# facebookresearch/moolib

Measured on AMD Instinct MI355X. Metric: env frames/sec (whole node) IMPALA Atari-ResNet, higher is better.
Workload: dtype bf16; 1 GPU; model=IMPALA Atari deep ResNet (16/32/32ch, FC3872-256), global_batch=32, seq_len=20, parallelism=dp1, actor_batch_size=128, num_actor_batches=2, num_actor_cpus=10, virtual_batch_size=32, num_actions=18, frame=84x84x4 uint8

## Files before the change

### csrc/accumulator.cc

```cpp
#include "accumulator.h"

#include <ATen/Functions.h>
#include <c10/core/GradMode.h>

#include <cstdlib>
#include <sstream>

namespace mrl {

namespace {
struct NoGrad {
  c10::AutoGradMode g{false};
};
}

Accumulator::Ptr Accumulator::create(std::string name, std::vector<at::Tensor> params,
                                     std::vector<at::Tensor> buffers,
                                     std::shared_ptr<Group> group) {
  Ptr p(new Accumulator(std::move(name), std::move(params), std::move(buffers), std::move(group)));
  p->setup();
  return p;
}

Accumulator::Accumulator(std::string name, std::vector<at::Tensor> params,
                         std::vector<at::Tensor> buffers, std::shared_ptr<Group> group)
    : name_(std::move(name)),
      allParams_(std::move(params)),
      buffers_(std::move(buffers)),
      group_(std::move(group)) {
  rpc_ = group_->rpc();
  for (auto& p : allParams_) {
    if (p.requires_grad()) params_.push_back(p);
  }
  int64_t total = 0;
  for (auto& p : params_) {
    offsets_.push_back(total);
    numels_.push_back(p.numel());
    total += p.numel();
  }
  slots_.resize(1);
  slots_[0].flat = makeFlatLocked();
  if (const char* e = getenv("MOOLIB_AMD_MODEL_BCAST_S")) {
    modelBcastInterval_ = atof(e);
  }
}

at::Tensor Accumulator::makeFlatLocked() {
  NoGrad ng;
  int64_t total = offsets_.empty() ? 1 : offsets_.back() + numels_.back();
  auto opts = params_.empty()
                  ? at::TensorOptions().dtype(at::kFloat)
                  : at::TensorOptions().dtype(params_[0].scalar_type()).device(params_[0].device());
  return at::zeros({std::max<int64_t>(total, 1)}, opts);
}

Accumulator::~Accumulator() {
  if (rpc_ && !rpc_->isShutdown()) {
    rpc_->undefine(fn("reqmodel"));
    rpc_->undefine(fn("modelupd"));
    rpc_->undefine(fn("buffers"));
  }
}

void Accumulator::setup() {
  std::weak_ptr<Accumulator> weak = weak_from_this();

  rpc_->define(fn("reqmodel"), [weak](Frame f, const std::string& from, RespondFn respond) {
    if (auto self = weak.lock()) {
      std::lock_guard<std::mutex> lk(self->mu_);
      if (std::find(self->stateRequesters_.begin(), self->stateRequesters_.end(), from) ==
          self->stateRequesters_.end()) {
        self->stateRequesters_.push_back(from);
      }
    }
    respond("", {}, false);
  });

  rpc_->define(fn("modelupd"), [weak](Frame f, const std::string& from, RespondFn respond) {
    auto self = weak.lock();
    if (!self) {
      respond("accumulator gone", {}, true);
      return;
    }
    try {
      WireReader r(f.payload);
      int64_t version = r.i64();
      uint32_t nParams = r.u32();
      uint32_t nBuffers = r.u32();
      std::string statePayload(r.str());
      if (uint64_t(nParams) > f.tensors.size() || uint64_t(nBuffers) > f.tensors.size() ||
          uint64_t(nParams) + uint64_t(nBuffers) > f.tensors.size())
        throw RpcError("model update tensor shortfall");
      std::lock_guard<std::mutex> lk(self->mu_);
      self->pendingParams_.assign(f.tensors.begin(), f.tensors.begin() + nParams);
      self->pendingBuffers_.assign(f.tensors.begin() + nParams,
                                   f.tensors.begin() + nParams + nBuffers);
      self->pendingStateTensors_.assign(f.tensors.begin() + nParams + nBuffers, f.tensors.end());
      self->pendingStatePayload_ = std::move(statePayload);
      self->pendingVersion_ = version;
      self->havePendingModel_ = true;
      respond("", {}, false);
    } catch (const std::exception& e) {
      respond(e.what(), {}, true);
    }
  });

  rpc_->define(fn("buffers"), [weak](Frame f, const std::string& from, RespondFn respond) {
    if (auto self = weak.lock()) {
      std::lock_guard<std::mutex> lk(self->mu_);
      if (f.tensors.size() == self->buffers_.size()) {
        NoGrad ng;
        for (size_t i = 0; i < self->buffers_.size(); ++i) {
          if (self->buffers_[i].sizes() == f.tensors[i].sizes()) {
            self->buffers_[i].copy_(f.tensors[i]);
          }
        }
      }
    }
    respond("", {}, false);
  });
}

void Accumulator::connect(const std::string& addr) { rpc_->connect(addr); }

void Accumulator::resetLocked(const char* why) {
  MRL_LOG_INFO("accumulator '%s': reset (%s)", name_.c_str(), why);
  epoch_++;
  decided_ = false;
  hasGradients_ = false;
  results_.clear();
  slotCursor_ = 0;
  hookLaunchCounter_ = 0;
  hookLaunchedUpTo_ = 0;
  for (auto& s : slots_) {
    s.newBatch = s.newGrads = s.newSkipped = 0;
    s.totBatch = s.totGrads = s.totSkipped = 0;
    s.phase = GradPhase::wantDecision;
    s.hookPending = false;
    if (s.hookPoll) {
      drains_.push_back(std::move(s.hookPoll));
      s.hookPoll = nullptr;
      s.flat = makeFlatLocked();
    } else {
      NoGrad ng;
      s.flat.zero_();
    }
  }
  havePendingModel_ = false;
  hasNewState_ = false;
  stateRequesters_.clear();
  modelRequestSent_ = false;
  leader_.clear();
  isLeader_ = false;
}

void Accumulator::failAndResyncLocked(const char* why) {
  MRL_LOG_INFO("accumulator '%s': %s; resync", name_.c_str(), why);
  phase_ = Phase::inactive;
  syncSeen_ = 0;
  group_->requestResync();
}

void Accumulator::startElectionLocked() {
  phase_ = Phase::electing;
  ReduceValue v;
  v.kind = ReduceValue::leaderTuple;
  v.version = modelVersion_;
  v.leaderName = group_->myName();
  uint64_t epoch = epoch_;
  std::weak_ptr<Accumulator> weak = weak_from_this();
  group_->allReduce(fn("elect"), std::move(v), nullptr,
                    [weak, epoch](ReduceValue* rv, const std::string* err) {
                      auto self = weak.lock();
                      if (!self) return;
                      std::lock_guard<std::mutex> lk(self->mu_);
                      if (epoch != self->epoch_ || self->phase_ != Phase::electing) return;
                      if (err) {
                        self->failAndResyncLocked(("election failed: " + *err).c_str());
                        return;
                      }
                      self->leader_ = rv->leaderName;
                      self->isLeader_ = (rv->leaderName == self->group_->myName());
                      MRL_LOG_INFO("accumulator '%s': leader is '%s' (version %lld)%s",
                                   self->name_.c_str(), self->leader_.c_str(),
                                   (long long)rv->version, self->isLeader_ ? " - that's me" : "");
                      if (self->isLeader_) {
                        self->phase_ = Phase::running;
                      } else {
                        self->phase_ = Phase::fetching;
                        self->modelRequestSent_ = false;
                      }
                    });
}

void Accumulator::update() {
  group_->update();
  bool active = group_->active();
  uint64_t sid = group_->syncId();

  std::vector<std::function<bool()>> pollTombs;
  std::unique_lock<std::mutex> lk(mu_);
  for (auto it = drains_.begin(); it != drains_.end();) {
    bool done = true;
    try {
      done = (*it)();
    } catch (const std::exception& e) {
      MRL_LOG_ERROR("abandoned hook drain failed: %s", e.what());
    }
    if (done) {
      pollTombs.push_back(std::move(*it));
      it = drains_.erase(it);
    } else {
      ++it;
    }
  }

  if (!active) {
    if (phase_ != Phase::inactive) resetLocked("group inactive");
    phase_ = Phase::inactive;
    syncSeen_ = 0;
    return;
  }
  if (sid != syncSeen_) {
    syncSeen_ = sid;
    resetLocked("membership changed");
    startElectionLocked();
    return;
  }

  if (phase_ == Phase::fetching) {
    if (!modelRequestSent_ || secondsSince(fetchStarted_) > 5.0) {
      modelRequestSent_ = true;
      fetchStarted_ = now();
      std::string leader = leader_;
      rpc_->sendRequest(leader, fn("reqmodel"), "", {},
                        [](Frame* resp, const std::string* err) {
                          if (err) MRL_LOG_VERBOSE("requestModel failed: %s", err->c_str());
                        },
                        10.0);
    }
  }

  if (havePendingModel_ && (phase_ == Phase::fetching || phase_ == Phase::running)) {
    NoGrad ng;
    bool shapesOk = pendingParams_.size() == allParams_.size() &&
                    pendingBuffers_.size() == buffers_.size();
    if (shapesOk) {
      for (size_t i = 0; i < allParams_.size(); ++i) {
        allParams_[i].copy_(pendingParams_[i], true);
      }
      for (size_t i = 0; i < buffers_.size(); ++i) {
        buffers_[i].copy_(pendingBuffers_[i], true);
      }
      modelVersion_ = pendingVersion_;
      hasNewState_ = !pendingStatePayload_.empty() || !pendingStateTensors_.empty();
      phase_ = Phase::running;
      MRL_LOG_INFO("accumulator '%s': model adopted at version %lld", name_.c_str(),
                   (long long)modelVersion_);
    } else {
      MRL_LOG_ERROR("accumulator '%s': model update shape mismatch — ignored", name_.c_str());
    }
    havePendingModel_ = false;
    pendingParams_.clear();
    pendingBuffers_.clear();
  }

  if (phase_ == Phase::running) {
    for (auto& s : slots_) {
      if (s.phase == GradPhase::reducing && secondsSince(s.started) > 120.0) {
        MRL_LOG_ERROR("accumulator '%s': gradient reduce wedged >120s", name_.c_str());
        failAndResyncLocked("reduce wedged");
        return;
      }
    }
    GradSlot& cur = slots_[slotCursor_];
    if (cur.phase == GradPhase::wantDecision && decided_) {
      startCountRoundLocked();
    }
    tryLaunchHooksLocked();
    for (size_t si = 0; si < slots_.size(); ++si) {
      GradSlot& s = slots_[si];
      if (s.phase == GradPhase::reducing && s.hookPoll && !s.hookPending) {
        bool done = false;
        try {
          done = s.hookPoll();
        } catch (const std::exception& e) {
          pollTombs.push_back(std::move(s.hookPoll));
          s.hookPoll = nullptr;
          MRL_LOG_ERROR("local reduce hook poll failed: %s", e.what());
          failAndResyncLocked("hook poll failed");
          return;
        }
        if (done) {
          pollTombs.push_back(std::move(s.hookPoll));
          s.hookPoll = nullptr;
          NoGrad ng;
          at::Tensor result = s.flat.clone();
          completeSlotLocked(si, std::move(result));
        }
      }
    }
    applyPendingLocked();
    maybeSendModelUpdatesLocked();
  }
}

void Accumulator::startCountRoundLocked() {
  size_t si = slotCursor_;
  GradSlot& s = slots_[si];
  s.phase = GradPhase::counting;
  s.started = now();
  ReduceValue v;
  v.kind = ReduceValue::counts;
  v.batchSize = s.newBatch;
  v.numGradients = s.newGrads;
  v.numSkipped = s.newSkipped;
  s.newBatch = s.newGrads = s.newSkipped = 0;
  uint64_t epoch = epoch_;
  std::weak_ptr<Accumulator> weak = weak_from_this();
  group_->allReduce(
      fn("count") + "/" + std::to_string(si), std::move(v), nullptr,
      [weak, epoch, si](ReduceValue* rv, const std::string* err) {
        auto self = weak.lock();
        if (!self) return;
        std::lock_guard<std::mutex> lk(self->mu_);
        if (epoch != self->epoch_) return;
        GradSlot& s = self->slots_[si];
        if (s.phase != GradPhase::counting) return;
        if (err) {
          self->failAndResyncLocked(("count round failed: " + *err).c_str());
          return;
        }
        s.totBatch += rv->batchSize;
        s.totGrads += rv->numGradients;
        s.totSkipped += rv->numSkipped;
        self->decided_ = false;
        if (s.totBatch >= self->virtualBatchSize_ && s.totGrads > 0) {
          self->enterReducingLocked(si);
        } else {
          s.phase = GradPhase::wantDecision;
        }
      });
}

void Accumulator::enterReducingLocked(size_t si) {
  GradSlot& s = slots_[si];
  s.phase = GradPhase::reducing;
  s.started = now();
  slotCursor_ = (si + 1) % slots_.size();
  if (hook_) {
    s.launchSeq = hookLaunchCounter_++;
    s.hookPending = true;
    tryLaunchHooksLocked();
    return;
  }
  ReduceValue v;
  v.kind = ReduceValue::gradBundle;
  {
    NoGrad ng;
    v.tensors.push_back(s.flat.device().is_cpu() ? s.flat.clone() : s.flat.to(at::kCPU));
  }
  uint64_t epoch = epoch_;
  std::weak_ptr<Accumulator> weak = weak_from_this();
  group_->allReduce(
      fn("grads") + "/" + std::to_string(si), std::move(v), nullptr,
      [weak, epoch, si](ReduceValue* rv, const std::string* err) {
        auto self = weak.lock();
        if (!self) return;
        std::lock_guard<std::mutex> lk(self->mu_);
        if (epoch != self->epoch_) return;
        GradSlot& s = self->slots_[si];
        if (s.phase != GradPhase::reducing) return;
        if (err) {
          self->failAndResyncLocked(("gradient reduce failed: " + *err).c_str());
          return;
        }
        NoGrad ng;
        at::Tensor result = rv->tensors.at(0);
        if (!s.flat.device().is_cpu()) result = result.to(s.flat.device(), true);
        self->completeSlotLocked(si, std::move(result));
      });
}

void Accumulator::tryLaunchHooksLocked() {
  if (!hook_ || !drains_.empty()) return;
  for (size_t si = 0; si < slots_.size(); ++si) {
    GradSlot& s = slots_[si];
    if (s.phase == GradPhase::reducing && s.hookPending && s.launchSeq == hookLaunchedUpTo_) {
      s.hookPending = false;
      ++hookLaunchedUpTo_;
      try {
        s.hookPoll = hook_(s.flat);
      } catch (const std::exception& e) {
        MRL_LOG_ERROR("local reduce hook failed: %s", e.what());
        failAndResyncLocked("hook launch failed");
        return;
      }
    }
  }
}

void Accumulator::completeSlotLocked(size_t si, at::Tensor result) {
  GradSlot& s = slots_[si];
  results_.push_back(PendingResult{std::move(result), s.totBatch, s.totGrads, s.totSkipped});
  s.totBatch = s.totGrads = s.totSkipped = 0;
  s.phase = GradPhase::wantDecision;
  {
    NoGrad ng;
    s.flat.zero_();
  }
}

void Accumulator::applyPendingLocked() {
  if (hasGradients_ || results_.empty()) return;
  PendingResult r = std::move(results_.front());
  results_.pop_front();
  NoGrad ng;
  int64_t n = std::max<int64_t>(r.grads, 1);
  r.flat.div_(static_cast<double>(n));
  for (size_t i = 0; i < params_.size(); ++i) {
    auto& p = params_[i];
    at::Tensor slice = r.flat.narrow(0, offsets_[i], numels_[i]).view(p.sizes());
    if (!p.grad().defined()) {
      p.mutable_grad() = slice.clone();
    } else {
      p.grad().copy_(slice, true);
    }
  }
  statBatch_ = r.batch;
  statGrads_ = r.grads;
  statSkipped_ = r.skipped;
  modelVersion_ += 1;
  hasGradients_ = true;
}

void Accumulator::maybeSendModelUpdatesLocked() {
  if (!isLeader_) return;
  if (!buffers_.empty() && secondsSince(lastBuffersBroadcast_) >= 10.0) {
    lastBuffersBroadcast_ = now();
    std::vector<at::Tensor> cpuBuffers;
    {
      NoGrad ng;
      for (auto& b : buffers_) cpuBuffers.push_back(b.detach().to(at::kCPU));
    }
    for (auto& m : group_->members()) {
      if (m == group_->myName()) continue;
      rpc_->sendRequest(m, fn("buffers"), "", cpuBuffers,
                        [](Frame*, const std::string*) {}, 10.0);
    }
  }
  if (lastModelBroadcast_.time_since_epoch().count() == 0) lastModelBroadcast_ = now();
  if (secondsSince(lastModelBroadcast_) >= modelBcastInterval_) {
    lastModelBroadcast_ = now();
    std::vector<at::Tensor> frameTensors;
    {
      NoGrad ng;
      for (auto& p : allParams_) frameTensors.push_back(p.detach().to(at::kCPU));
      for (auto& b : buffers_) frameTensors.push_back(b.detach().to(at::kCPU));
    }
    WireWriter w;
    w.i64(modelVersion_);
    w.u32(static_cast<uint32_t>(allParams_.size()));
    w.u32(static_cast<uint32_t>(buffers_.size()));
    w.str("");
    for (auto& m : group_->members()) {
      if (m == group_->myName()) continue;
      rpc_->sendRequest(m, fn("modelupd"), w.out, frameTensors,
                        [](Frame*, const std::string*) {}, 30.0);
    }
  }
}

bool Accumulator::connected() {
  std::lock_guard<std::mutex> lk(mu_);
  return phase_ == Phase::running;
}

bool Accumulator::wantsState() {
  std::lock_guard<std::mutex> lk(mu_);
  return phase_ == Phase::running && isLeader_ && !stateRequesters_.empty();
}

bool Accumulator::hasNewState() {
  std::lock_guard<std::mutex> lk(mu_);
  return hasNewState_;
}

void Accumulator::setState(std::string payload, std::vector<at::Tensor> tensors) {
  std::vector<std::string> requesters;
  int64_t version;
  std::vector<at::Tensor> frameTensors;
  uint32_t nParams, nBuffers;
  {
    std::lock_guard<std::mutex> lk(mu_);
    requesters.swap(stateRequesters_);
    version = modelVersion_;
    NoGrad ng;
    for (auto& p : allParams_) frameTensors.push_back(p.detach().to(at::kCPU));
    for (auto& b : buffers_) frameTensors.push_back(b.detach().to(at::kCPU));
    nParams = static_cast<uint32_t>(allParams_.size());
    nBuffers = static_cast<uint32_t>(buffers_.size());
  }
  for (auto& t : tensors) frameTensors.push_back(t.device().is_cpu() ? t : t.to(at::kCPU));
  WireWriter w;
  w.i64(version);
  w.u32(nParams);
  w.u32(nBuffers);
  w.str(payload);
  for (auto& r : requesters) {
    rpc_->sendRequest(r, fn("modelupd"), w.out, frameTensors,
                      [r](Frame*, const std::string* err) {
                        if (err) {
                          MRL_LOG_INFO("model update to '%s' failed: %s", r.c_str(), err->c_str());
                        }
                      },
                      30.0);
  }
}

std::pair<std::string, std::vector<at::Tensor>> Accumulator::state() {
  std::lock_guard<std::mutex> lk(mu_);
  hasNewState_ = false;
  return {pendingStatePayload_, pendingStateTensors_};
}

bool Accumulator::wantsGradients() {
  std::lock_guard<std::mutex> lk(mu_);
  if (phase_ != Phase::running || decided_) return false;
  if (slots_[slotCursor_].phase != GradPhase::wantDecision) return false;
  size_t pending = results_.size() + (hasGradients_ ? 1 : 0);
  return pending < slots_.size();
}

bool Accumulator::hasGradients() {
  std::lock_guard<std::mutex> lk(mu_);
  return hasGradients_;
}

void Accumulator::skipGradients() {
  std::lock_guard<std::mutex> lk(mu_);
  if (phase_ != Phase::running || decided_) return;
  GradSlot& s = slots_[slotCursor_];
  if (s.phase != GradPhase::wantDecision) return;
  decided_ = true;
  s.newSkipped += 1;
}

void Accumulator::reduceGradients(int64_t batchSize) {
  std::lock_guard<std::mutex> lk(mu_);
  GradSlot& s = slots_[slotCursor_];
  if (phase_ != Phase::running || s.phase != GradPhase::wantDecision || decided_) {
    throw RpcError("reduce_gradients called when wants_gradients() is false");
  }
  NoGrad ng;
  std::vector<at::Tensor> slices, flatGrads, grads;
  slices.reserve(params_.size());
  flatGrads.reserve(params_.size());
  grads.reserve(params_.size());
  for (size_t i = 0; i < params_.size(); ++i) {
    auto& p = params_[i];
    if (p.grad().defined()) {
      slices.push_back(s.flat.narrow(0, offsets_[i], numels_[i]));
      flatGrads.push_back(p.grad().flatten());
      grads.push_back(p.grad());
    }
  }
  if (!grads.empty()) {
    at::_foreach_add_(slices, flatGrads);
    at::_foreach_zero_(grads);
  }
  decided_ = true;
  s.newBatch += batchSize;
  s.newGrads += 1;
}

void Accumulator::zeroGradients() {
  std::lock_guard<std::mutex> lk(mu_);
  NoGrad ng;
  std::vector<at::Tensor> grads;
  for (auto& p : params_) {
    if (p.grad().defined()) grads.push_back(p.grad());
  }
  if (!grads.empty()) at::_foreach_zero_(grads);
  hasGradients_ = false;
  applyPendingLocked();
}

int64_t Accumulator::modelVersion() {
  std::lock_guard<std::mutex> lk(mu_);
  return modelVersion_;
}

void Accumulator::setModelVersion(int64_t v) {
  std::lock_guard<std::mutex> lk(mu_);
  modelVersion_ = v;
}

std::string Accumulator::getLeader() {
  std::lock_guard<std::mutex> lk(mu_);
  return leader_;
}

bool Accumulator::isLeader() {
  std::lock_guard<std::mutex> lk(mu_);
  return isLeader_;
}

std::unordered_map<std::string, int64_t> Accumulator::gradientStats() {
  std::lock_guard<std::mutex> lk(mu_);
  return {{"batch_size", statBatch_}, {"num_gradients", statGrads_}, {"num_skipped", statSkipped_}};
}

void Accumulator::setVirtualBatchSize(int64_t n) {
  std::lock_guard<std::mutex> lk(mu_);
  virtualBatchSize_ = std::max<int64_t>(n, 1);
}

void Accumulator::setParallelGradients(int64_t n) {
  std::lock_guard<std::mutex> lk(mu_);
  n = std::max<int64_t>(n, 1);
  if (static_cast<size_t>(n) == slots_.size()) return;
  slots_.resize(n);
  for (auto& s : slots_) {
    if (!s.flat.defined()) s.flat = makeFlatLocked();
  }
}

void Accumulator::setLocalReduceHook(LocalReduceHook h) {
  LocalReduceHook old;
  {
    std::lock_guard<std::mutex> lk(mu_);
    old = std::move(hook_);
    hook_ = std::move(h);
  }
}

std::string Accumulator::debugState() {
  std::lock_guard<std::mutex> lk(mu_);
  std::ostringstream os;
  os << "Accumulator '" << name_ << "' phase=" << static_cast<int>(phase_)
     << " leader='" << leader_ << "' version=" << modelVersion_ << " decided=" << decided_
     << " cursor=" << slotCursor_ << " hasGrads=" << hasGradients_
     << " results=" << results_.size() << " slots=[";
  for (auto& s : slots_) {
    os << static_cast<int>(s.phase) << "(tb=" << s.totBatch << ")";
  }
  os << "]";
  return os.str();
}

}
```

### csrc/accumulator.h

```cpp
#pragma once

#include <deque>

#include "services.h"

namespace mrl {

class Accumulator : public std::enable_shared_from_this<Accumulator> {
 public:
  using Ptr = std::shared_ptr<Accumulator>;
  using LocalReduceHook = std::function<std::function<bool()>(at::Tensor&)>;

  static Ptr create(std::string name, std::vector<at::Tensor> params,
                    std::vector<at::Tensor> buffers, std::shared_ptr<Group> group);
  ~Accumulator();

  void connect(const std::string& addr);
  void update();
  bool connected();

  bool wantsState();
  bool hasNewState();
  void setState(std::string payload, std::vector<at::Tensor> tensors);
  std::pair<std::string, std::vector<at::Tensor>> state();

  bool wantsGradients();
  bool hasGradients();
  void skipGradients();
  void reduceGradients(int64_t batchSize);
  void zeroGradients();

  int64_t modelVersion();
  void setModelVersion(int64_t v);
  std::string getLeader();
  bool isLeader();
  std::unordered_map<std::string, int64_t> gradientStats();

  void setVirtualBatchSize(int64_t n);
  void setParallelGradients(int64_t n);
  void setLocalReduceHook(LocalReduceHook h);

  std::shared_ptr<Group> group() { return group_; }
  std::string debugState();

 private:
  Accumulator(std::string name, std::vector<at::Tensor> params, std::vector<at::Tensor> buffers,
              std::shared_ptr<Group> group);
  void setup();

  enum class Phase { inactive, electing, fetching, running };
  enum class GradPhase { wantDecision, counting, reducing, resultReady };

  struct GradSlot {
    at::Tensor flat;
    int64_t newBatch = 0, newGrads = 0, newSkipped = 0;
    int64_t totBatch = 0, totGrads = 0, totSkipped = 0;
    GradPhase phase = GradPhase::wantDecision;
    std::function<bool()> hookPoll;
    uint64_t launchSeq = 0;
    bool hookPending = false;
    TimePoint started{};
  };
  struct PendingResult {
    at::Tensor flat;
    int64_t batch, grads, skipped;
  };

  void resetLocked(const char* why);
  void startElectionLocked();
  void startCountRoundLocked();
  void enterReducingLocked(size_t si);
  void tryLaunchHooksLocked();
  void completeSlotLocked(size_t si, at::Tensor result);
  void applyPendingLocked();
  void failAndResyncLocked(const char* why);
  at::Tensor makeFlatLocked();
  void maybeSendModelUpdatesLocked();
  std::string fn(const char* suffix) const { return "__mrl_acc_" + std::string(suffix) + ":" + name_; }

  std::string name_;
  std::vector<at::Tensor> params_;
  std::vector<at::Tensor> allParams_;
  std::vector<at::Tensor> buffers_;
  std::shared_ptr<Group> group_;
  RpcPtr rpc_;

  std::mutex mu_;
  Phase phase_ = Phase::inactive;
  GradPhase gradPhase_ = GradPhase::wantDecision;
  uint64_t syncSeen_ = 0;
  uint64_t epoch_ = 0;
  int64_t modelVersion_ = 0;
  std::string leader_;
  bool isLeader_ = false;
  TimePoint fetchStarted_{};
  bool modelRequestSent_ = false;

  bool havePendingModel_ = false;
  int64_t pendingVersion_ = 0;
  std::vector<at::Tensor> pendingParams_, pendingBuffers_;
  std::string pendingStatePayload_;
  std::vector<at::Tensor> pendingStateTensors_;
  bool hasNewState_ = false;

  std::vector<std::string> stateRequesters_;
  TimePoint lastBuffersBroadcast_{};
  TimePoint lastModelBroadcast_{};
  double modelBcastInterval_ = 600.0;

  std::vector<GradSlot> slots_;
  size_t slotCursor_ = 0;
  std::vector<int64_t> offsets_, numels_;
  int64_t virtualBatchSize_ = 1;
  bool decided_ = false;
  bool hasGradients_ = false;
  int64_t statBatch_ = 0, statGrads_ = 0, statSkipped_ = 0;
  std::deque<PendingResult> results_;
  LocalReduceHook hook_;
  uint64_t hookLaunchCounter_ = 0;
  uint64_t hookLaunchedUpTo_ = 0;
  std::vector<std::function<bool()>> drains_;
};

}
```

### csrc/services.cc

```cpp
#include "services.h"

#include <algorithm>

namespace mrl {


void ReduceValue::encode(WireWriter& w) const {
  w.u8(static_cast<uint8_t>(kind));
  switch (kind) {
    case pyObject:
      w.str(payload);
      break;
    case counts:
      w.i64(batchSize);
      w.i64(numGradients);
      w.i64(numSkipped);
      break;
    case gradBundle:
      w.i64(batchSize);
      w.i64(numGradients);
      w.i64(numSkipped);
      break;
    case leaderTuple:
      w.i64(version);
      w.str(leaderName);
      break;
  }
}

ReduceValue ReduceValue::decode(WireReader& r, std::vector<at::Tensor> tensors) {
  ReduceValue v;
  v.kind = static_cast<Kind>(r.u8());
  switch (v.kind) {
    case pyObject:
      v.payload = std::string(r.str());
      v.tensors = std::move(tensors);
      break;
    case counts:
      v.batchSize = r.i64();
      v.numGradients = r.i64();
      v.numSkipped = r.i64();
      break;
    case gradBundle:
      v.batchSize = r.i64();
      v.numGradients = r.i64();
      v.numSkipped = r.i64();
      v.tensors = std::move(tensors);
      break;
    case leaderTuple:
      v.version = r.i64();
      v.leaderName = std::string(r.str());
      break;
  }
  return v;
}

void ReduceValue::fold(ReduceValue& src, const std::function<void(ReduceValue&, ReduceValue&)>& pyFold) {
  if (src.kind != kind) throw RpcError("allreduce: mismatched value kinds");
  switch (kind) {
    case pyObject:
      if (!pyFold) throw RpcError("allreduce: missing fold op for python values");
      pyFold(*this, src);
      break;
    case counts:
      batchSize += src.batchSize;
      numGradients += src.numGradients;
      numSkipped += src.numSkipped;
      break;
    case gradBundle:
      batchSize += src.batchSize;
      numGradients += src.numGradients;
      numSkipped += src.numSkipped;
      if (tensors.size() != src.tensors.size())
        throw RpcError("allreduce: gradient bundle tensor count mismatch");
      for (size_t i = 0; i < tensors.size(); ++i) {
        if (!tensors[i].sizes().equals(src.tensors[i].sizes()))
          throw RpcError("allreduce: gradient tensor shape mismatch at index " + std::to_string(i));
        tensors[i].add_(src.tensors[i]);
      }
      break;
    case leaderTuple:
      if (std::tie(src.version, src.leaderName) > std::tie(version, leaderName)) {
        version = src.version;
        leaderName = src.leaderName;
      }
      break;
  }
}


namespace {
constexpr const char* kBrokerPing = "__mrl_broker_ping";
constexpr const char* kBrokerResync = "__mrl_broker_resync";
}

void Broker::GroupState::resort() {
  if (!dirty) return;
  dirty = false;
  sortedCache.clear();
  std::vector<std::pair<std::pair<int64_t, uint64_t>, std::string>> v;
  for (auto& [name, m] : members) v.push_back({{m.sortOrder, m.joinSeq}, name});
  std::sort(v.begin(), v.end());
  for (auto& e : v) sortedCache.push_back(e.second);
}

Broker::Broker(RpcPtr rpc) : rpc_(std::move(rpc)) {
  rpc_->define(kBrokerResync, [this](Frame f, const std::string& fromPeer, RespondFn respond) {
    try {
      WireReader r(f.payload);
      std::string group(r.str());
      std::lock_guard<std::mutex> lk(mu_);
      if (secondsSince(lastForcedResync_) > 0.5) {
        lastForcedResync_ = now();
        auto it = groups_.find(group);
        if (it != groups_.end()) {
          it->second.syncId++;
          it->second.dirty = true;
          it->second.resort();
          MRL_LOG_INFO("broker: forced resync of group '%s' by '%s' (syncId now %llu)",
                       group.c_str(), fromPeer.c_str(), (unsigned long long)it->second.syncId);
        }
      }
      respond("", {}, false);
    } catch (const std::exception& e) {
      respond(e.what(), {}, true);
    }
  });
  rpc_->define(kBrokerPing, [this](Frame f, const std::string& fromPeer, RespondFn respond) {
    try {
      WireReader r(f.payload);
      std::string group(r.str());
      std::string member(r.str());
      int64_t sortOrder = r.i64();
      double timeout = r.f64();
      (void)fromPeer;
      WireWriter w;
      {
        std::lock_guard<std::mutex> lk(mu_);
        GroupState& g = groups_[group];
        if (timeout > 0) g.timeout = timeout;
        evictStaleLocked(g);
        auto it = g.members.find(member);
        if (it == g.members.end()) {
          Member m;
          m.lastPing = now();
          m.sortOrder = sortOrder;
          m.joinSeq = g.joinCounter++;
          g.members[member] = m;
          g.syncId++;
          g.dirty = true;
          MRL_LOG_INFO("broker: '%s' joined group '%s' (syncId now %llu, %zu members)",
                       member.c_str(), group.c_str(), (unsigned long long)g.syncId,
                       g.members.size());
        } else {
          it->second.lastPing = now();
          if (it->second.sortOrder != sortOrder) {
            it->second.sortOrder = sortOrder;
            g.syncId++;
            g.dirty = true;
          }
        }
        g.resort();
        w.u64(g.syncId);
        w.u32(static_cast<uint32_t>(g.sortedCache.size()));
        for (auto& n : g.sortedCache) w.str(n);
      }
      respond(std::move(w.out), {}, false);
    } catch (const std::exception& e) {
      respond(std::string("broker error: ") + e.what(), {}, true);
    }
  });
}

Broker::~Broker() {
  if (rpc_ && !rpc_->isShutdown()) {
    rpc_->undefine(kBrokerPing);
    rpc_->undefine(kBrokerResync);
  }
}

void Broker::setName(const std::string& n) { rpc_->setName(n); }
void Broker::listen(const std::string& addr) { rpc_->listen(addr); }

void Broker::evictStaleLocked(GroupState& g) {
  for (auto it = g.members.begin(); it != g.members.end();) {
    if (secondsSince(it->second.lastPing) > g.timeout) {
      MRL_LOG_INFO("broker: evicting stale member '%s'", it->first.c_str());
      it = g.members.erase(it);
      g.syncId++;
      g.dirty = true;
    } else {
      ++it;
    }
  }
  g.resort();
}

void Broker::update() {
  std::lock_guard<std::mutex> lk(mu_);
  for (auto& [name, g] : groups_) evictStaleLocked(g);
}


std::shared_ptr<Group> Group::create(RpcPtr rpc, std::string name) {
  std::shared_ptr<Group> g(new Group(std::move(rpc), std::move(name)));
  g->setup();
  return g;
}

Group::Group(RpcPtr rpc, std::string name) : rpc_(std::move(rpc)), name_(std::move(name)) {}

void Group::setup() {
  std::weak_ptr<Group> weak = shared_from_this();
  rpc_->define(funcUp(), [weak](Frame f, const std::string& from, RespondFn respond) {
    if (auto g = weak.lock()) g->handleContribution(false, f, from, respond);
  });
  rpc_->define(funcDown(), [weak](Frame f, const std::string& from, RespondFn respond) {
    if (auto g = weak.lock()) g->handleContribution(true, f, from, respond);
  });
}

Group::~Group() {
  std::vector<AllReduceOpPtr> toFail;
  {
    std::lock_guard<std::mutex> lk(mu_);
    stopped_ = true;
    for (auto& [k, op] : ops_) {
      if (op->done && !op->completed) {
        op->completed = true;
        toFail.push_back(op);
      }
    }
    ops_.clear();
  }
  for (auto& op : toFail) {
    std::string err = "group destroyed";
    op->done(nullptr, &err);
  }
  if (rpc_ && !rpc_->isShutdown()) {
    rpc_->undefine(funcUp());
    rpc_->undefine(funcDown());
  }
}

std::vector<std::string> Group::members() {
  std::lock_guard<std::mutex> lk(mu_);
  return members_;
}
uint64_t Group::syncId() {
  std::lock_guard<std::mutex> lk(mu_);
  return syncId_;
}
bool Group::active() {
  std::lock_guard<std::mutex> lk(mu_);
  return active_;
}

void Group::update() {
  bool sendPing = false;
  {
    std::lock_guard<std::mutex> lk(mu_);
    double interval = active_ ? 0.5 : 0.2;
    if (!pingInFlight_ && secondsSince(lastPing_) >= interval) {
      pingInFlight_ = true;
      lastPing_ = now();
      sendPing = true;
    }
  }
  if (sendPing) {
    WireWriter w;
    w.str(name_);
    w.str(myName());
    w.i64(sortOrder_.load());
    w.f64(timeout_.load());
    std::weak_ptr<Group> weak = shared_from_this();
    rpc_->sendRequest(
        brokerName_, kBrokerPing, std::move(w.out), {},
        [weak](Frame* resp, const std::string* error) {
          auto g = weak.lock();
          if (!g) return;
          std::vector<std::pair<AllReduceOpPtr, OpKey>> toAdvance;
          std::vector<AllReduceOpPtr> toFail;
          std::string failMsg;
          {
            std::lock_guard<std::mutex> lk(g->mu_);
            g->pingInFlight_ = false;
            if (error) {
              if (g->active_ && secondsSince(g->lastPingOk_) > g->timeout_.load()) {
                g->active_ = false;
                MRL_LOG_INFO("group '%s': lost contact with broker (%s)", g->name_.c_str(),
                             error->c_str());
              } else if (!g->active_ && g->lastPingOk_.time_since_epoch().count() == 0 &&
                         secondsSince(g->lastUnreachableWarn_) > 10.0) {
                g->lastUnreachableWarn_ = now();
                MRL_LOG_ERROR(
                    "group '%s': cannot reach broker peer '%s' (%s) — check the broker's "
                    "rpc name and connect() address",
                    g->name_.c_str(), g->brokerName_.c_str(), error->c_str());
              }
              return;
            }
            g->lastPingOk_ = now();
            WireReader r(resp->payload);
            uint64_t syncId = r.u64();
            uint32_t n = r.u32();
            std::vector<std::string> members;
            for (uint32_t i = 0; i < n; ++i) members.emplace_back(r.str());
            bool inGroup =
                std::find(members.begin(), members.end(), g->myName()) != members.end();
            if (syncId != g->syncId_) {
              MRL_LOG_INFO("group '%s': syncId %llu -> %llu (%u members)", g->name_.c_str(),
                           (unsigned long long)g->syncId_, (unsigned long long)syncId, n);
              for (auto it = g->ops_.begin(); it != g->ops_.end();) {
                if (it->first.syncId < syncId) {
                  auto op = it->second;
                  if (!op->completed) {
                    op->completed = true;
                    if (op->done) toFail.push_back(op);
                  }
                  it = g->ops_.erase(it);
                } else {
                  ++it;
                }
              }
              failMsg = "group membership changed (syncId " + std::to_string(g->syncId_) +
                        " -> " + std::to_string(syncId) + ")";
              g->syncId_ = syncId;
              g->members_ = members;
              g->seqByName_.clear();
              g->active_ = inGroup;
              for (auto& [key, op] : g->ops_) {
                if (key.syncId == syncId && op->childrenExpected < 0) {
                  op->members = members;
                  auto mit = std::find(members.begin(), members.end(), g->myName());
                  op->myIndex = mit == members.end() ? -1 : int(mit - members.begin());
                  int n2 = static_cast<int>(members.size());
                  int c = 0;
                  if (op->myIndex >= 0) {
                    if (2 * op->myIndex + 1 < n2) ++c;
                    if (2 * op->myIndex + 2 < n2) ++c;
                  }
                  op->childrenExpected = c;
                  toAdvance.push_back({op, key});
                }
              }
            } else {
              g->active_ = inGroup;
            }
          }
          for (auto& op : toFail) op->done(nullptr, &failMsg);
          for (auto& [op, key] : toAdvance) g->advance(key, op);
        },
        timeout_.load());
  }
  std::vector<AllReduceOpPtr> timedOut;
  {
    std::lock_guard<std::mutex> lk(mu_);
    for (auto it = ops_.begin(); it != ops_.end();) {
      if (!it->second->completed && now() >= it->second->deadline) {
        it->second->completed = true;
        if (it->second->done) timedOut.push_back(it->second);
        it = ops_.erase(it);
      } else {
        ++it;
      }
    }
  }
  std::string err = "allreduce timed out";
  for (auto& op : timedOut) op->done(nullptr, &err);
}

void Group::requestResync() {
  WireWriter w;
  w.str(name_);
  rpc_->sendRequest(brokerName_, kBrokerResync, std::move(w.out), {},
                    [](Frame*, const std::string*) {}, 10.0);
}

void Group::allReduce(const std::string& opName, ReduceValue value, PyFold fold, ReduceDone done) {
  OpKey key;
  AllReduceOpPtr op;
  {
    std::lock_guard<std::mutex> lk(mu_);
    if (!active_) {
      std::string err = "group not active";
      op = nullptr;
      key = {};
      globalScheduler().run([done = std::move(done), err] { done(nullptr, &err); });
      return;
    }
    key.syncId = syncId_;
    key.opName = opName;
    key.seq = seqByName_[opName]++;
    auto& slot = ops_[key];
    if (!slot) slot = std::make_shared<AllReduceOp>();
    op = slot;
    op->localContributed = true;
    op->acc = std::move(value);
    op->pyFold = std::move(fold);
    op->done = std::move(done);
    op->deadline = now() + std::chrono::duration_cast<Clock::duration>(
                               std::chrono::duration<double>(timeout_.load()));
    op->members = members_;
    auto mit = std::find(members_.begin(), members_.end(), myName());
    op->myIndex = mit == members_.end() ? -1 : int(mit - members_.begin());
    int n = static_cast<int>(members_.size());
    int c = 0;
    if (op->myIndex >= 0) {
      if (2 * op->myIndex + 1 < n) ++c;
      if (2 * op->myIndex + 2 < n) ++c;
    }
    op->childrenExpected = c;
  }
  advance(key, op);
}

void Group::advance(const OpKey& key, AllReduceOpPtr op) {
  while (true) {
    std::vector<std::pair<std::string, ReduceValue>> batch;
    bool sendUpNow = false;
    bool completeNow = false;
    {
      std::lock_guard<std::mutex> lk(mu_);
      if (op->completed || op->folding || !op->localContributed || op->childrenExpected < 0) return;
      if (op->sentUp) return;
      if (!op->queued.empty()) {
        batch = std::move(op->queued);
        op->queued.clear();
        op->folding = true;
      } else if (op->childrenArrived >= op->childrenExpected && !op->sentUp) {
        op->sentUp = true;
        if (op->myIndex == 0) {
          completeNow = true;
        } else {
          sendUpNow = true;
        }
      } else {
        return;
      }
    }
    if (!batch.empty()) {
      std::string foldError;
      for (auto& [from, v] : batch) {
        try {
          op->acc->fold(v, op->pyFold);
        } catch (const std::exception& e) {
          foldError = e.what();
          break;
        }
      }
      {
        std::lock_guard<std::mutex> lk(mu_);
        op->folding = false;
        op->childrenArrived += static_cast<int>(batch.size());
      }
      if (!foldError.empty()) {
        completeOp(key, op, nullptr, "allreduce fold failed: " + foldError);
        return;
      }
      continue;
    }
    if (sendUpNow) {
      int parent = (op->myIndex - 1) / 2;
      sendValue(op->members[parent], false, key, *op->acc);
      return;
    }
    if (completeNow) {
      ReduceValue result = *op->acc;
      int n = static_cast<int>(op->members.size());
      if (2 * op->myIndex + 1 < n) sendValue(op->members[2 * op->myIndex + 1], true, key, result);
      if (2 * op->myIndex + 2 < n) sendValue(op->members[2 * op->myIndex + 2], true, key, result);
      completeOp(key, op, &result, "");
      return;
    }
  }
}

void Group::completeOp(const OpKey& key, AllReduceOpPtr op, ReduceValue* v, const std::string& err) {
  {
    std::lock_guard<std::mutex> lk(mu_);
    if (op->completed) return;
    op->completed = true;
    ops_.erase(key);
  }
  if (op->done) {
    if (v) {
      auto val = std::make_shared<ReduceValue>(std::move(*v));
      for (auto& t : val->tensors) t = t.clone();
      globalScheduler().run([done = std::move(op->done), val] { done(val.get(), nullptr); });
    } else {
      globalScheduler().run([done = std::move(op->done), err] { done(nullptr, &err); });
    }
  }
}

void Group::sendValue(const std::string& member, bool isDown, const OpKey& key,
                      const ReduceValue& v) {
  WireWriter w;
  w.u64(key.syncId);
  w.u64(key.seq);
  w.str(key.opName);
  v.encode(w);
  std::string groupName = name_;
  rpc_->sendRequest(
      member, isDown ? funcDown() : funcUp(), std::move(w.out), v.tensors,
      [groupName, member](Frame* resp, const std::string* error) {
        if (error) {
          MRL_LOG_VERBOSE("group '%s': send to '%s' failed: %s", groupName.c_str(),
                          member.c_str(), error->c_str());
        }
      },
      timeout_.load());
}

void Group::handleContribution(bool isDown, Frame& f, const std::string& from, RespondFn respond) {
  respond("", {}, false);
  try {
    WireReader r(f.payload);
    OpKey key;
    key.syncId = r.u64();
    key.seq = r.u64();
    key.opName = std::string(r.str());
    ReduceValue v = ReduceValue::decode(r, std::move(f.tensors));

    AllReduceOpPtr op;
    bool isRootResult = false;
    {
      std::lock_guard<std::mutex> lk(mu_);
      if (stopped_) return;
      if (key.syncId < syncId_) return;
      auto& slot = ops_[key];
      if (!slot) {
        slot = std::make_shared<AllReduceOp>();
        slot->deadline = now() + std::chrono::duration_cast<Clock::duration>(
                                     std::chrono::duration<double>(timeout_.load()));
        if (key.syncId == syncId_) {
          slot->members = members_;
          auto mit = std::find(members_.begin(), members_.end(), myName());
          slot->myIndex = mit == members_.end() ? -1 : int(mit - members_.begin());
          int n = static_cast<int>(members_.size());
          int c = 0;
          if (slot->myIndex >= 0) {
            if (2 * slot->myIndex + 1 < n) ++c;
            if (2 * slot->myIndex + 2 < n) ++c;
          }
          slot->childrenExpected = c;
        }
      }
      op = slot;
      if (!isDown) {
        op->queued.push_back({from, std::move(v)});
      } else {
        isRootResult = true;
      }
    }
    if (isRootResult) {
      std::vector<std::string> fwd;
      {
        std::lock_guard<std::mutex> lk(mu_);
        if (op->completed) return;
        int n = static_cast<int>(op->members.size());
        if (op->myIndex >= 0) {
          if (2 * op->myIndex + 1 < n) fwd.push_back(op->members[2 * op->myIndex + 1]);
          if (2 * op->myIndex + 2 < n) fwd.push_back(op->members[2 * op->myIndex + 2]);
        }
      }
      for (auto& m : fwd) sendValue(m, true, key, v);
      completeOp(key, op, &v, "");
    } else {
      advance(key, op);
    }
  } catch (const std::exception& e) {
    MRL_LOG_ERROR("group '%s': bad contribution: %s", name_.c_str(), e.what());
  }
}

}
```

### csrc/services.h

```cpp
#pragma once

#include <optional>

#include "rpc.h"

namespace mrl {


struct ReduceValue {
  enum Kind : uint8_t { pyObject = 0, counts = 1, gradBundle = 2, leaderTuple = 3 };
  Kind kind = pyObject;
  std::string payload;
  std::vector<at::Tensor> tensors;
  int64_t batchSize = 0;
  int64_t numGradients = 0;
  int64_t numSkipped = 0;
  int64_t version = 0;
  std::string leaderName;

  void encode(WireWriter& w) const;
  static ReduceValue decode(WireReader& r, std::vector<at::Tensor> tensors);
  void fold(ReduceValue& src, const std::function<void(ReduceValue&, ReduceValue&)>& pyFold);
};

using PyFold = std::function<void(ReduceValue& dst, ReduceValue& src)>;

using ReduceDone = std::function<void(ReduceValue* value, const std::string* error)>;


class Broker {
 public:
  explicit Broker(RpcPtr rpc);
  ~Broker();
  void setName(const std::string& n);
  void listen(const std::string& addr);
  void update();

 private:
  TimePoint lastForcedResync_{};
  struct Member {
    TimePoint lastPing{};
    int64_t sortOrder = 0;
    uint64_t joinSeq = 0;
  };
  struct GroupState {
    std::unordered_map<std::string, Member> members;
    uint64_t syncId = 1;
    uint64_t joinCounter = 0;
    double timeout = 6.0;
    std::vector<std::string> sortedCache;
    bool dirty = true;
    void resort();
  };
  void evictStaleLocked(GroupState& g);
  RpcPtr rpc_;
  std::mutex mu_;
  std::unordered_map<std::string, GroupState> groups_;
};


struct OpKey {
  uint64_t syncId;
  uint64_t seq;
  std::string opName;
  bool operator==(const OpKey& o) const {
    return syncId == o.syncId && seq == o.seq && opName == o.opName;
  }
};
struct OpKeyHash {
  size_t operator()(const OpKey& k) const {
    return std::hash<uint64_t>()(k.syncId * 1000003 + k.seq) ^ std::hash<std::string>()(k.opName);
  }
};

struct AllReduceOp {
  std::optional<ReduceValue> acc;
  int childrenArrived = 0;
  int childrenExpected = -1;
  bool localContributed = false;
  bool sentUp = false;
  bool completed = false;
  bool folding = false;
  std::vector<std::pair<std::string, ReduceValue>> queued;
  PyFold pyFold;
  ReduceDone done;
  TimePoint deadline{};
  std::vector<std::string> members;
  int myIndex = -1;
};
using AllReduceOpPtr = std::shared_ptr<AllReduceOp>;

class Group : public std::enable_shared_from_this<Group> {
 public:
  static std::shared_ptr<Group> create(RpcPtr rpc, std::string name);
  ~Group();

  void update();
  void setBrokerName(const std::string& n) { brokerName_ = n; }
  void setTimeout(double t) { timeout_ = t; }
  void setSortOrder(int64_t o) { sortOrder_ = o; }
  std::vector<std::string> members();
  uint64_t syncId();
  const std::string& name() const { return name_; }
  bool active();

  void allReduce(const std::string& opName, ReduceValue value, PyFold fold, ReduceDone done);

  void requestResync();

  RpcPtr rpc() { return rpc_; }
  std::string myName() { return rpc_->getName(); }

 private:
  Group(RpcPtr rpc, std::string name);
  void setup();

  void handleContribution(bool isDown, Frame& f, const std::string& from, RespondFn respond);
  void advance(const OpKey& key, AllReduceOpPtr op);
  void completeOp(const OpKey& key, AllReduceOpPtr op, ReduceValue* v, const std::string& err);
  void sendValue(const std::string& member, bool isDown, const OpKey& key, const ReduceValue& v);
  std::string funcUp() const { return "__mrl_group_up:" + name_; }
  std::string funcDown() const { return "__mrl_group_down:" + name_; }

  RpcPtr rpc_;
  std::string name_;
  std::string brokerName_ = "broker";
  std::atomic<double> timeout_{10.0};
  std::atomic<int64_t> sortOrder_{0};

  std::mutex mu_;
  std::vector<std::string> members_;
  uint64_t syncId_ = 0;
  bool active_ = false;
  bool pingInFlight_ = false;
  TimePoint lastPing_{};
  TimePoint lastPingOk_{};
  TimePoint lastUnreachableWarn_{};
  std::unordered_map<std::string, uint64_t> seqByName_;
  std::unordered_map<OpKey, AllReduceOpPtr, OpKeyHash> ops_;
  bool stopped_ = false;
};

}
```

Baseline: 82770 frames/s.

## Skip tree all-reduce for single-member groups and use flat gradient views

When the group has only this process as member, a gradient round is completed locally: the accumulated bucket is handed over directly and swapped with a fresh zeroed buffer, instead of copying to CPU and running the RPC all-reduce tree. When all parameter grads are contiguous aliases of one flat storage, accumulation, zeroing and the final divide are done as single ops on that flat view instead of per-parameter foreach calls. Counters for local, tree, hook and flat rounds are added to the status string. Risk: correctness depends on the membership check matching syncSeen_, and the flat path only triggers if grads already share one storage.

Result: faster. 95320 frames/s, median of 5 (+15.2%).

```diff
diff --git a/csrc/accumulator.cc b/csrc/accumulator.cc
--- a/csrc/accumulator.cc
+++ b/csrc/accumulator.cc
@@ -1,6 +1,8 @@
 #include "accumulator.h"
 
 #include <ATen/Functions.h>
+#include <ATen/ScalarOps.h>
+#include <c10/core/DeviceGuard.h>
 #include <c10/core/GradMode.h>
 
 #include <cstdlib>
@@ -137,6 +139,7 @@
     s.totBatch = s.totGrads = s.totSkipped = 0;
     s.phase = GradPhase::wantDecision;
     s.hookPending = false;
+    s.localPending = false;
     if (s.hookPoll) {
       drains_.push_back(std::move(s.hookPoll));
       s.hookPoll = nullptr;
@@ -280,6 +283,10 @@
     tryLaunchHooksLocked();
     for (size_t si = 0; si < slots_.size(); ++si) {
       GradSlot& s = slots_[si];
+      if (s.phase == GradPhase::reducing && s.localPending) {
+        completeLocalLocked(si);
+        continue;
+      }
       if (s.phase == GradPhase::reducing && s.hookPoll && !s.hookPending) {
         bool done = false;
         try {
@@ -351,9 +358,15 @@
   if (hook_) {
     s.launchSeq = hookLaunchCounter_++;
     s.hookPending = true;
+    ++hookRounds_;
     tryLaunchHooksLocked();
     return;
   }
+  if (soloRoundLocked(s)) {
+    s.localPending = true;
+    return;
+  }
+  ++treeRounds_;
   ReduceValue v;
   v.kind = ReduceValue::gradBundle;
   {
@@ -400,12 +413,32 @@
   }
 }
 
-void Accumulator::completeSlotLocked(size_t si, at::Tensor result) {
+bool Accumulator::soloRoundLocked(const GradSlot& s) {
+  if (hook_) return false;
+  if (s.totBatch < virtualBatchSize_ || s.totGrads <= 0) return false;
+  auto [sid, members] = group_->membership();
+  return sid == syncSeen_ && members.size() == 1 && members[0] == group_->myName();
+}
+
+void Accumulator::completeLocalLocked(size_t si) {
+  GradSlot& s = slots_[si];
+  NoGrad ng;
+  c10::OptionalDeviceGuard guard;
+  if (!s.flat.device().is_cpu()) guard.reset_device(s.flat.device());
+  at::Tensor fresh = at::zeros_like(s.flat);
+  s.localPending = false;
+  at::Tensor result = std::move(s.flat);
+  s.flat = std::move(fresh);
+  ++localRounds_;
+  completeSlotLocked(si, std::move(result), false);
+}
+
+void Accumulator::completeSlotLocked(size_t si, at::Tensor result, bool zeroBucket) {
   GradSlot& s = slots_[si];
   results_.push_back(PendingResult{std::move(result), s.totBatch, s.totGrads, s.totSkipped});
   s.totBatch = s.totGrads = s.totSkipped = 0;
   s.phase = GradPhase::wantDecision;
-  {
+  if (zeroBucket) {
     NoGrad ng;
     s.flat.zero_();
   }
@@ -417,14 +450,20 @@
   results_.pop_front();
   NoGrad ng;
   int64_t n = std::max<int64_t>(r.grads, 1);
-  r.flat.div_(static_cast<double>(n));
-  for (size_t i = 0; i < params_.size(); ++i) {
-    auto& p = params_[i];
-    at::Tensor slice = r.flat.narrow(0, offsets_[i], numels_[i]).view(p.sizes());
-    if (!p.grad().defined()) {
-      p.mutable_grad() = slice.clone();
-    } else {
-      p.grad().copy_(slice, true);
+  at::Tensor view = flatGradViewLocked();
+  if (view.defined()) {
+    at::div_out(view, r.flat, at::native::wrapped_scalar_tensor(static_cast<double>(n)));
+    ++flatCalls_;
+  } else {
+    r.flat.div_(static_cast<double>(n));
+    for (size_t i = 0; i < params_.size(); ++i) {
+      auto& p = params_[i];
+      at::Tensor slice = r.flat.narrow(0, offsets_[i], numels_[i]).view(p.sizes());
+      if (!p.grad().defined()) {
+        p.mutable_grad() = slice.clone();
+      } else {
+        p.grad().copy_(slice, true);
+      }
     }
   }
   statBatch_ = r.batch;
@@ -553,21 +592,28 @@
     throw RpcError("reduce_gradients called when wants_gradients() is false");
   }
   NoGrad ng;
-  std::vector<at::Tensor> slices, flatGrads, grads;
-  slices.reserve(params_.size());
-  flatGrads.reserve(params_.size());
-  grads.reserve(params_.size());
-  for (size_t i = 0; i < params_.size(); ++i) {
-    auto& p = params_[i];
-    if (p.grad().defined()) {
-      slices.push_back(s.flat.narrow(0, offsets_[i], numels_[i]));
-      flatGrads.push_back(p.grad().flatten());
-      grads.push_back(p.grad());
-    }
-  }
-  if (!grads.empty()) {
-    at::_foreach_add_(slices, flatGrads);
-    at::_foreach_zero_(grads);
+  at::Tensor view = flatGradViewLocked();
+  if (view.defined()) {
+    s.flat.add_(view);
+    view.zero_();
+    ++flatCalls_;
+  } else {
+    std::vector<at::Tensor> slices, flatGrads, grads;
+    slices.reserve(params_.size());
+    flatGrads.reserve(params_.size());
+    grads.reserve(params_.size());
+    for (size_t i = 0; i < params_.size(); ++i) {
+      auto& p = params_[i];
+      if (p.grad().defined()) {
+        slices.push_back(s.flat.narrow(0, offsets_[i], numels_[i]));
+        flatGrads.push_back(p.grad().flatten());
+        grads.push_back(p.grad());
+      }
+    }
+    if (!grads.empty()) {
+      at::_foreach_add_(slices, flatGrads);
+      at::_foreach_zero_(grads);
+    }
   }
   decided_ = true;
   s.newBatch += batchSize;
@@ -577,13 +623,39 @@
 void Accumulator::zeroGradients() {
   std::lock_guard<std::mutex> lk(mu_);
   NoGrad ng;
-  std::vector<at::Tensor> grads;
-  for (auto& p : params_) {
-    if (p.grad().defined()) grads.push_back(p.grad());
-  }
-  if (!grads.empty()) at::_foreach_zero_(grads);
+  at::Tensor view = flatGradViewLocked();
+  if (view.defined()) {
+    view.zero_();
+    ++flatCalls_;
+  } else {
+    std::vector<at::Tensor> grads;
+    for (auto& p : params_) {
+      if (p.grad().defined()) grads.push_back(p.grad());
+    }
+    if (!grads.empty()) at::_foreach_zero_(grads);
+  }
   hasGradients_ = false;
   applyPendingLocked();
+}
+
+at::Tensor Accumulator::flatGradViewLocked() {
+  if (params_.empty()) return {};
+  const at::Tensor& flat = slots_[0].flat;
+  const at::Tensor& g0 = params_[0].grad();
+  if (!g0.defined()) return {};
+  const int64_t base = g0.storage_offset();
+  for (size_t i = 0; i < params_.size(); ++i) {
+    const at::Tensor& g = params_[i].grad();
+    if (!g.defined() || g.scalar_type() != flat.scalar_type() || g.device() != flat.device() ||
+        g.layout() != at::kStrided || g.numel() != numels_[i] || !g.is_contiguous() ||
+        !g.is_alias_of(g0) || g.storage_offset() != base + offsets_[i]) {
+      return {};
+    }
+  }
+  const int64_t total = offsets_.back() + numels_.back();
+  if (total <= 0) return {};
+  NoGrad ng;
+  return at::as_strided(g0, {total}, {1}, base);
 }
 
 int64_t Accumulator::modelVersion() {
@@ -646,6 +718,8 @@
     os << static_cast<int>(s.phase) << "(tb=" << s.totBatch << ")";
   }
   os << "]";
+  os << " local_rounds=" << localRounds_ << " tree_rounds=" << treeRounds_
+     << " hook_rounds=" << hookRounds_ << " flat_calls=" << flatCalls_;
   return os.str();
 }
 
diff --git a/csrc/accumulator.h b/csrc/accumulator.h
--- a/csrc/accumulator.h
+++ b/csrc/accumulator.h
@@ -59,6 +59,7 @@
     std::function<bool()> hookPoll;
     uint64_t launchSeq = 0;
     bool hookPending = false;
+    bool localPending = false;
     TimePoint started{};
   };
   struct PendingResult {
@@ -71,7 +72,10 @@
   void startCountRoundLocked();
   void enterReducingLocked(size_t si);
   void tryLaunchHooksLocked();
-  void completeSlotLocked(size_t si, at::Tensor result);
+  bool soloRoundLocked(const GradSlot& s);
+  void completeLocalLocked(size_t si);
+  at::Tensor flatGradViewLocked();
+  void completeSlotLocked(size_t si, at::Tensor result, bool zeroBucket = true);
   void applyPendingLocked();
   void failAndResyncLocked(const char* why);
   at::Tensor makeFlatLocked();
@@ -120,6 +124,11 @@
   uint64_t hookLaunchCounter_ = 0;
   uint64_t hookLaunchedUpTo_ = 0;
   std::vector<std::function<bool()>> drains_;
+
+  uint64_t localRounds_ = 0;
+  uint64_t treeRounds_ = 0;
+  uint64_t hookRounds_ = 0;
+  uint64_t flatCalls_ = 0;
 };
 
 }
diff --git a/csrc/services.cc b/csrc/services.cc
--- a/csrc/services.cc
+++ b/csrc/services.cc
@@ -250,6 +250,10 @@
 uint64_t Group::syncId() {
   std::lock_guard<std::mutex> lk(mu_);
   return syncId_;
+}
+std::pair<uint64_t, std::vector<std::string>> Group::membership() {
+  std::lock_guard<std::mutex> lk(mu_);
+  return {syncId_, members_};
 }
 bool Group::active() {
   std::lock_guard<std::mutex> lk(mu_);
diff --git a/csrc/services.h b/csrc/services.h
--- a/csrc/services.h
+++ b/csrc/services.h
@@ -101,6 +101,7 @@
   void setSortOrder(int64_t o) { sortOrder_ = o; }
   std::vector<std::string> members();
   uint64_t syncId();
+  std::pair<uint64_t, std::vector<std::string>> membership();
   const std::string& name() const { return name_; }
   bool active();
 
```
